# david-wb/tiny-diffusion

Measured on AMD Instinct MI355X. Metric: train images/s (q_sample+fwd+MSE+bwd+allreduce+Adam), MNIST 28x28 UNet fp32; 1000-step sample latency in `sample`, higher is better.
Workload: dtype f32; 1 GPU; diffusion.py unconditional MNIST 28x28 UNet, fp32, train step, batch 256/GPU (BASELINE.json configs[1]); global_batch=256, per_gpu_batch=256, parallelism=dp1

## Files before the change

### tiny_diffusion_amd/csrc/conv3x3_wino.hip

```cpp
#include "internal.h"
#include "conv_shared.h"


constexpr int WT = 64;
constexpr int WN = 64;
constexpr int WK = 8;
constexpr int A_ST = 16 * WT * WK;
constexpr int B_ST = 16 * WN * WK;
constexpr int STAGE = A_ST + B_ST;

struct WinoArgs {
  const float* in;
  const float* u;
  const float* bias;
  float* out;
  const float* out_scale;
  const float* out_shift;
  float* stats;
  int B, H, W, Cin, Cout, th, tw, NT, tilesN, M;
  float rcp_tpi, rcp_tw;
  int per;
  int compact;
  unsigned long long* stamps;
};

constexpr int OLD = 68;
constexpr int TAB_OFF = 2 * STAGE;
typedef unsigned u32x4 __attribute__((ext_vector_type(4)));

template <int EPI, int XH = -1>
__device__ __forceinline__ void wino_epilogue(const WinoArgs& a, float* out, const float* bias, f32x16 (&acc)[16], float* smem,
                                              int tblk, int n0, int wm, int wn, int l31, int half, int tid,
                                              const f32x4* xin = nullptr) {
#if defined(__HIP_DEVICE_COMPILE__)
  const unsigned* tab = reinterpret_cast<const unsigned*>(smem + TAB_OFF);
  const int cl = wn * 32 + l31, col = n0 + cl;
  const float bv = bias ? bias[col] : 0.f;
  float osc = 1.f, osh = 0.f;
  if (EPI == EPI_BNRELU) { osc = a.out_scale[col]; osh = a.out_shift[col]; }
  float csum = 0.f, cnt = 0.f;
  float* ot = smem;
  f32x4 pv[8];
#pragma unroll
  for (int r = 0; r < 16; ++r) {
    if (XH >= 0 && (r & 3) == 0) {
#pragma unroll
      for (int p = 0; p < 8; ++p) pv[p] = xin[(p * 4 + (r >> 2)) * 64];
    }
    auto M = [&](int p) { return XH >= 0 && (p >> 3) != XH ? pv[p & 7][r & 3] : acc[p][r]; };
    float s0[4], s1[4];
#pragma unroll
    for (int nu = 0; nu < 4; ++nu) {
      s0[nu] = M(0 + nu) + M(4 + nu) + M(8 + nu);
      s1[nu] = M(4 + nu) - M(8 + nu) - M(12 + nu);
    }
    float y[4] = {s0[0] + s0[1] + s0[2], s0[1] - s0[2] - s0[3], s1[0] + s1[1] + s1[2], s1[1] - s1[2] - s1[3]};
    const int tl = wm * 32 + (r & 3) + 8 * (r >> 2) + 4 * half;
    const unsigned m = tab[2 * tl + 1];
#pragma unroll
    for (int q = 0; q < 4; ++q) {
      float val = y[q] + bv;
      if (EPI == EPI_BNRELU) val = fmaxf(fmaf(val, osc, osh), 0.f);
      const bool ok = (m >> q) & 1u;
      if (XH < 0) ot[(tl * 4 + q) * OLD + cl] = val;
      csum += ok ? val : 0.f;
      cnt += ok ? 1.f : 0.f;
      y[q] = ok ? val : 0.f;
    }
    acc[0][r] = y[0]; acc[1][r] = y[1]; acc[4][r] = y[2]; acc[5][r] = y[3];
    acc[2][r] = (m & 1u) ? 1.f : 0.f;
    acc[3][r] = (m & 2u) ? 1.f : 0.f;
    acc[6][r] = (m & 4u) ? 1.f : 0.f;
    acc[7][r] = (m & 8u) ? 1.f : 0.f;
  }
  if (XH >= 0) {
    __syncthreads();
#pragma unroll
    for (int r = 0; r < 16; ++r) {
      const int tl = wm * 32 + (r & 3) + 8 * (r >> 2) + 4 * half;
      ot[(tl * 4 + 0) * OLD + cl] = acc[0][r]; ot[(tl * 4 + 1) * OLD + cl] = acc[1][r];
      ot[(tl * 4 + 2) * OLD + cl] = acc[4][r]; ot[(tl * 4 + 3) * OLD + cl] = acc[5][r];
    }
  }
  __syncthreads();
  {
    const auto rsrc_out = __builtin_amdgcn_make_buffer_rsrc(out, 0, (int)((int64_t)a.M * a.Cout * 4), 0x00020000);
    const int c4 = (tid & 15) * 4, q = (tid >> 4) & 3;
    const unsigned qoff = (unsigned)((((q >> 1) * a.W + (q & 1)) * a.Cout + n0 + c4) * 4);
    const uint2* tab2 = reinterpret_cast<const uint2*>(tab);
    const float* src = ot + (tid >> 4) * OLD + c4;
#pragma unroll
    for (int i = 0; i < 16; ++i) {
      const uint2 e = tab2[4 * i + (tid >> 6)];
      const unsigned off = ((e.y >> q) & 1u) ? e.x + qoff : 0x80000000u;
      const f32x4 v = *reinterpret_cast<const f32x4*>(src + i * 16 * OLD);
      __builtin_amdgcn_raw_buffer_store_b128(__builtin_bit_cast(u32x4, v), rsrc_out, off, 0, 0);
    }
  }
  if (EPI == EPI_STATS) {
    float* red = smem + 256 * OLD;
    const float s = csum + __shfl_xor(csum, 32, 64);
    const float n = cnt + __shfl_xor(cnt, 32, 64);
    if (half == 0) { red[wm * 64 + cl] = s; red[128 + wm * 64 + cl] = n; }
    __syncthreads();
    if (tid < 64) {
      const float ts = red[tid] + red[64 + tid];
      const float tn = red[128 + tid] + red[192 + tid];
      red[256 + tid] = tn > 0.f ? ts / tn : 0.f;
      a.stats[((size_t)tblk * 2 + 0) * a.Cout + n0 + tid] = ts;
    }
    __syncthreads();
    const float mean = red[256 + cl];
    float q = 0.f;
#pragma unroll
    for (int r = 0; r < 16; ++r) {
      const float d0 = acc[0][r] - mean, d1 = acc[1][r] - mean, d2 = acc[4][r] - mean, d3 = acc[5][r] - mean;
      q = fmaf(d0 * acc[2][r], d0, q); q = fmaf(d1 * acc[3][r], d1, q);
      q = fmaf(d2 * acc[6][r], d2, q); q = fmaf(d3 * acc[7][r], d3, q);
    }
    q += __shfl_xor(q, 32, 64);
    __syncthreads();
    if (half == 0) red[wm * 64 + cl] = q;
    __syncthreads();
    if (tid < 64) a.stats[((size_t)tblk * 2 + 1) * a.Cout + n0 + tid] = red[tid] + red[64 + tid];
  }
#endif
}

#if defined(__HIP_DEVICE_COMPILE__)
__device__ __forceinline__ float s_add(float x, float y) { float r; asm("v_add_f32 %0, %1, %2" : "=v"(r) : "v"(x), "v"(y)); return r; }
__device__ __forceinline__ float s_sub(float x, float y) { float r; asm("v_sub_f32 %0, %1, %2" : "=v"(r) : "v"(x), "v"(y)); return r; }
__device__ __forceinline__ f32x4 add4(f32x4 x, f32x4 y) { return f32x4{s_add(x[0], y[0]), s_add(x[1], y[1]), s_add(x[2], y[2]), s_add(x[3], y[3])}; }
__device__ __forceinline__ f32x4 sub4(f32x4 x, f32x4 y) { return f32x4{s_sub(x[0], y[0]), s_sub(x[1], y[1]), s_sub(x[2], y[2]), s_sub(x[3], y[3])}; }
#endif

__device__ __forceinline__ int div_rcp(int n, int d, float r, int* rem) {
  int q = (int)((float)n * r);
  int m = n - q * d;
  if (m < 0) { --q; m += d; }
  else if (m >= d) { ++q; m -= d; }
  *rem = m;
  return q;
}

template <int EPI, bool SPLITK, bool ROWS>
__global__ void __launch_bounds__(256)
conv3x3_wino_kernel(WinoArgs a) {
#if defined(__HIP_DEVICE_COMPILE__)
  static_assert(!ROWS || (!SPLITK && EPI != EPI_BNRELU), "the row split serves the training launches only");
  typedef __attribute__((address_space(3))) void* lds_ptr_t;
  extern __shared__ __attribute__((aligned(16))) float smem[];
  const unsigned long long t_entry = a.stamps ? __builtin_amdgcn_s_memrealtime() : 0ull;
  const int tid = threadIdx.x;
  const int lane = tid & 63;
  const int wave = __builtin_amdgcn_readfirstlane(tid >> 6);
  const int l31 = lane & 31, half = lane >> 5;
  const int wm = ROWS ? wave & 1 : wave >> 1, wn = ROWS ? wave >> 1 : wave & 1;
  const int xb = blockIdx.x / (8 * a.tilesN), xr = blockIdx.x % (8 * a.tilesN);
  const int tblk = a.compact ? (int)blockIdx.x / a.tilesN : xb * 8 + (xr & 7);
  const int nblk = a.compact ? (int)blockIdx.x - tblk * a.tilesN : xr >> 3;
  const int T0 = tblk * WT;
  if (T0 >= a.NT) return;
  const int n0 = nblk * WN;
  const int tpi = a.th * a.tw;

  if (tid < WT) {
    const int T = T0 + tid;
    const bool tv = T < a.NT;
    int rem, tx;
    const int b = div_rcp(T, tpi, a.rcp_tpi, &rem);
    const int ty = div_rcp(rem, a.tw, a.rcp_tw, &tx);
    const bool r1 = 2 * ty + 1 < a.H, c1 = 2 * tx + 1 < a.W;
    unsigned* tab = reinterpret_cast<unsigned*>(smem + TAB_OFF);
    tab[2 * tid] = tv ? (unsigned)(((b * a.H + 2 * ty) * a.W + 2 * tx) * a.Cout * 4) : 0u;
    tab[2 * tid + 1] = tv ? (1u | (c1 ? 2u : 0u) | (r1 ? 4u : 0u) | (r1 && c1 ? 8u : 0u)) : 0u;
  }

  const auto rsrc_in = __builtin_amdgcn_make_buffer_rsrc(const_cast<float*>(a.in), 0, (int)((int64_t)a.M * a.Cin * 4), 0x00020000);
  const auto rsrc_u = __builtin_amdgcn_make_buffer_rsrc(const_cast<float*>(a.u), 0, a.Cout * 16 * a.Cin * 4, 0x00020000);
  constexpr unsigned OOB = 0x80000000u;
  unsigned a_off[4][2];
#pragma unroll
  for (int g = 0; g < 2; ++g) {
    const int T = T0 + g * 32 + (lane >> 1);
    const bool tv = T < a.NT;
    int rem, tx;
    const int b = div_rcp(T, tpi, a.rcp_tpi, &rem);
    const int ty = div_rcp(rem, a.tw, a.rcp_tw, &tx);
#pragma unroll
    for (int j = 0; j < 4; ++j) {
      const int px = 4 * wave + j;
      const int ih = 2 * ty - 1 + (px >> 2), iw = 2 * tx - 1 + (px & 3);
      const bool ok = tv && (unsigned)ih < (unsigned)a.H && (unsigned)iw < (unsigned)a.W;
      a_off[j][g] = ok ? (unsigned)((((b * a.H + ih) * a.W + iw) * a.Cin + (lane & 1) * 4) * 4) : OOB;
    }
  }
  const unsigned u_base = (unsigned)(nblk * (a.Cin / WK)) * (unsigned)(B_ST * 4) + (unsigned)(wave * 8 * 1024 + lane * 16);

  const int s0 = SPLITK ? (int)blockIdx.y * a.per : 0;
  const int ns = SPLITK ? min(a.per, a.Cin / WK - s0) : a.Cin / WK;
  auto piece = [&](int i, int buf, int k) {
    const int sc = s0 + (k < ns ? k : ns - 1);
    float* Ab = smem + buf * STAGE;
    float* Bb = Ab + A_ST;
    if (i < 8)
      __builtin_amdgcn_raw_ptr_buffer_load_lds(rsrc_u, (lds_ptr_t)(Bb + (wave * 8 + i) * 256), 16, u_base + i * 1024,
                                               (unsigned)sc * (unsigned)(B_ST * 4), 0, 0);
    else
      __builtin_amdgcn_raw_ptr_buffer_load_lds(rsrc_in, (lds_ptr_t)(Ab + (4 * wave + ((i - 8) >> 1)) * 512 + ((i - 8) & 1) * 256), 16,
                                               a_off[(i - 8) >> 1][(i - 8) & 1], (unsigned)(sc * WK * 4), 0, 0);
  };

  constexpr bool PEEL = !SPLITK && EPI != EPI_BNRELU;
  f32x16 acc[16];
  const f32x16 zero16 = {0.f, 0.f, 0.f, 0.f, 0.f, 0.f, 0.f, 0.f, 0.f, 0.f, 0.f, 0.f, 0.f, 0.f, 0.f, 0.f};
  if (!PEEL) {
#pragma unroll
    for (int p = 0; p < 16; ++p)
#pragma unroll
      for (int r = 0; r < 16; ++r) acc[p][r] = 0.f;
  }

#pragma unroll
  for (int i = 0; i < 16; ++i) piece(i, 0, 0);
  unsigned long long t_issued = 0, t_landed = 0, t_loop = 0, c_loop = 0;
  if constexpr (ROWS) {
    static_assert(4 * 8 * 16 * 64 == 2 * STAGE, "the exchange fills the ring");
#pragma unroll
    for (int i = 0; i < 8; ++i) piece(i, 1, 1);
    if (a.stamps) t_issued = __builtin_amdgcn_s_memrealtime();
    asm volatile("s_waitcnt vmcnt(8) lgkmcnt(0)\n\ts_barrier" ::: "memory");
    if (a.stamps) { t_landed = __builtin_amdgcn_s_memrealtime(); c_loop = __builtin_amdgcn_s_memtime(); }
    auto body = [&](auto Hc) {
      constexpr int H = decltype(Hc)::value;
      f32x4 d[12], v[8], t[4], bq[5], nbq[2];
      const int lofs = wm * 256 + l31 * 8 + half * 4;
      auto trow = [&](int x, int c) {
        if (H == 0) t[c] = x == 0 ? sub4(d[c], d[8 + c]) : add4(d[4 + c], d[8 + c]);
        else t[c] = x == 0 ? sub4(d[4 + c], d[c]) : sub4(d[c], d[8 + c]);
      };
      auto vcol = [&](int x, int c) {
        f32x4& o = v[4 * x + c];
        if (c == 0) o = sub4(t[0], t[2]);
        else if (c == 1) o = add4(t[1], t[2]);
        else if (c == 2) o = sub4(t[2], t[1]);
        else o = sub4(t[1], t[3]);
      };
      constexpr int RA = 0, RB = H == 0 ? 2 : 1, RC = H == 0 ? 1 : 2;
      {
        const float* Ab = smem + 4 * H * 512 + lofs;
        const float* Bb = smem + A_ST + 8 * H * 512 + l31 * 8 + half * 4;
#pragma unroll
        for (int c = 0; c < 4; ++c) {
          d[4 * RA + c] = *reinterpret_cast<const f32x4*>(Ab + (4 * RA + c) * 512);
          d[4 * RB + c] = *reinterpret_cast<const f32x4*>(Ab + (4 * RB + c) * 512);
        }
        nbq[0] = *reinterpret_cast<const f32x4*>(Bb);
        nbq[1] = *reinterpret_cast<const f32x4*>(Bb + 256);
#pragma unroll
        for (int c = 0; c < 4; ++c) d[4 * RC + c] = *reinterpret_cast<const f32x4*>(Ab + (4 * RC + c) * 512);
#pragma unroll
        for (int c = 0; c < 4; ++c) trow(0, c);
#pragma unroll
        for (int c = 0; c < 4; ++c) vcol(0, c);
      }
      auto stage = [&](auto first_c, int s) {
        constexpr bool FIRST = decltype(first_c)::value;
        const int cb = s & 1;
        const float* Bb = smem + cb * STAGE + A_ST + 8 * H * 512 + l31 * 8 + half * 4;
        const float* An = smem + (cb ^ 1) * STAGE + 4 * H * 512 + lofs;
        const float* Bn = smem + (cb ^ 1) * STAGE + A_ST + 8 * H * 512 + l31 * 8 + half * 4;
        bq[0] = nbq[0]; bq[1] = nbq[1];
        __builtin_amdgcn_sched_barrier(0);
#pragma unroll
        for (int g = 0; g < 16; ++g) {
          const int cur = g % 5, pp = g >> 1, ai = 8 * (g & 1) + pp;
          if (FIRST) acc[ai] = __builtin_amdgcn_mfma_f32_32x32x2f32(v[pp][0], bq[cur][0], zero16, 0, 0, 0);
          else acc[ai] = __builtin_amdgcn_mfma_f32_32x32x2f32(v[pp][0], bq[cur][0], acc[ai], 0, 0, 0);
          if (g < 8) piece(8 + g, cb ^ 1, s + 1);
          if (g == 10) bq[4] = *reinterpret_cast<const f32x4*>(Bb + 14 * 256);
          if (g == 11) bq[0] = *reinterpret_cast<const f32x4*>(Bb + 15 * 256);
          if (g == 12) {
            asm volatile("s_waitcnt vmcnt(0) lgkmcnt(0)\n\ts_barrier" ::: "memory");
#pragma unroll
            for (int c = 0; c < 4; ++c) {
              d[4 * RA + c] = *reinterpret_cast<const f32x4*>(An + (4 * RA + c) * 512);
              d[4 * RB + c] = *reinterpret_cast<const f32x4*>(An + (4 * RB + c) * 512);
            }
          }
          if (g == 13) {
#pragma unroll
            for (int c = 0; c < 4; ++c) d[4 * RC + c] = *reinterpret_cast<const f32x4*>(An + (4 * RC + c) * 512);
          }
          if (g == 14) {
#pragma unroll
            for (int c = 0; c < 4; ++c) trow(0, c);
          }
          if (g == 15) { vcol(0, 2); vcol(0, 3); }
          __builtin_amdgcn_sched_barrier(0);
          acc[ai] = __builtin_amdgcn_mfma_f32_32x32x2f32(v[pp][1], bq[cur][1], acc[ai], 0, 0, 0);
          if (g < 2) { trow(1, 2 * g); trow(1, 2 * g + 1); }
          else if (g < 4) { vcol(1, 2 * g - 4); vcol(1, 2 * g - 3); }
          else if (g >= 12) piece(2 * (g - 12), cb, s + 2);
          __builtin_amdgcn_sched_barrier(0);
          acc[ai] = __builtin_amdgcn_mfma_f32_32x32x2f32(v[pp][2], bq[cur][2], acc[ai], 0, 0, 0);
          if (g < 12) bq[(g + 2) % 5] = *reinterpret_cast<const f32x4*>(Bb + (g + 2) * 256);
          if (g == 12) { nbq[0] = *reinterpret_cast<const f32x4*>(Bn); nbq[1] = *reinterpret_cast<const f32x4*>(Bn + 256); }
          if (g == 14) { vcol(0, 0); vcol(0, 1); }
          if (g == 15) piece(7, cb, s + 2);
          __builtin_amdgcn_sched_barrier(0);
          acc[ai] = __builtin_amdgcn_mfma_f32_32x32x2f32(v[pp][3], bq[cur][3], acc[ai], 0, 0, 0);
          if (g >= 12 && g < 15) piece(2 * (g - 12) + 1, cb, s + 2);
          __builtin_amdgcn_sched_barrier(0);
        }
      };
      stage(std::true_type{}, 0);
      for (int s = 1; s < ns; ++s) stage(std::false_type{}, s);
      asm volatile("s_waitcnt vmcnt(0) lgkmcnt(0)\n\ts_barrier" ::: "memory");
      if (a.stamps) { t_loop = __builtin_amdgcn_s_memrealtime(); c_loop = __builtin_amdgcn_s_memtime() - c_loop; }
      {
        f32x4* xo = reinterpret_cast<f32x4*>(smem) + (2 * (1 - H) + wm) * 2048 + lane;
#pragma unroll
        for (int pp = 0; pp < 8; ++pp)
#pragma unroll
          for (int r4 = 0; r4 < 4; ++r4) {
            const f32x16& x = acc[8 * (1 - H) + pp];
            xo[(pp * 4 + r4) * 64] = f32x4{x[4 * r4], x[4 * r4 + 1], x[4 * r4 + 2], x[4 * r4 + 3]};
          }
      }
      __syncthreads();
      wino_epilogue<EPI, H>(a, a.out, a.bias, acc, smem, tblk, n0, wm, H, l31, half, tid,
                            reinterpret_cast<const f32x4*>(smem) + wave * 2048 + lane);
    };
    if (wn) body(std::integral_constant<int, 1>{});
    else body(std::integral_constant<int, 0>{});
  } else {
    f32x4 d[16], v[16], t1[4], t2[4], t3[4];
    auto xop = [&](int q) {
      const int r = q >> 3, k = q & 7, c = k & 3;
      if (k < 4) {
        if (r == 0) t1[c] = add4(d[4 + c], d[8 + c]);
        else if (r == 1) t2[c] = sub4(d[8 + c], d[4 + c]);
        else t3[c] = sub4(d[4 + c], d[12 + c]);
      } else {
        f32x4(&t)[4] = r == 0 ? t1 : r == 1 ? t2 : t3;
        f32x4& o = v[4 * (r + 1) + c];
        if (c == 0) o = sub4(t[0], t[2]);
        else if (c == 1) o = add4(t[1], t[2]);
        else if (c == 2) o = sub4(t[2], t[1]);
        else o = sub4(t[1], t[3]);
      }
    };
    {
#pragma unroll
      for (int i = 0; i < 8; ++i) piece(i, 1, 1);
      if (a.stamps) t_issued = __builtin_amdgcn_s_memrealtime();
      asm volatile("s_waitcnt vmcnt(8) lgkmcnt(0)\n\ts_barrier" ::: "memory");
      if (a.stamps) { t_landed = __builtin_amdgcn_s_memrealtime(); c_loop = __builtin_amdgcn_s_memtime(); }
      f32x4 bq[5], nbq[2];
      {
        const float* Ab = smem + wm * 256 + l31 * 8 + half * 4;
        const float* Bb = smem + A_ST + wn * 256 + l31 * 8 + half * 4;
#pragma unroll
        for (int c = 0; c < 4; ++c) { d[c] = *reinterpret_cast<const f32x4*>(Ab + c * 512); d[8 + c] = *reinterpret_cast<const f32x4*>(Ab + (8 + c) * 512); }
        nbq[0] = *reinterpret_cast<const f32x4*>(Bb);
        nbq[1] = *reinterpret_cast<const f32x4*>(Bb + 512);
#pragma unroll
        for (int c = 0; c < 4; ++c) { d[4 + c] = *reinterpret_cast<const f32x4*>(Ab + (4 + c) * 512); d[12 + c] = *reinterpret_cast<const f32x4*>(Ab + (12 + c) * 512); }
        f32x4 t0[4];
#pragma unroll
        for (int c = 0; c < 4; ++c) t0[c] = sub4(d[c], d[8 + c]);
        v[0] = sub4(t0[0], t0[2]); v[1] = add4(t0[1], t0[2]); v[2] = sub4(t0[2], t0[1]); v[3] = sub4(t0[1], t0[3]);
      }
      auto stage = [&](auto first_c, int s) {
        constexpr bool FIRST = decltype(first_c)::value;
        const int cb = s & 1;
        const float* Bb = smem + cb * STAGE + A_ST + wn * 256 + l31 * 8 + half * 4;
        const float* An = smem + (cb ^ 1) * STAGE + wm * 256 + l31 * 8 + half * 4;
        const float* Bn = smem + (cb ^ 1) * STAGE + A_ST + wn * 256 + l31 * 8 + half * 4;
        bq[0] = nbq[0]; bq[1] = nbq[1];
        __builtin_amdgcn_sched_barrier(0);
#pragma unroll
        for (int p = 0; p < 16; ++p) {
          const int cur = p % 5;
          if (FIRST) acc[p] = __builtin_amdgcn_mfma_f32_32x32x2f32(v[p][0], bq[cur][0], zero16, 0, 0, 0);
          else acc[p] = __builtin_amdgcn_mfma_f32_32x32x2f32(v[p][0], bq[cur][0], acc[p], 0, 0, 0);
          if (p < 8) piece(8 + p, cb ^ 1, s + 1);
          if (p == 10) bq[4] = *reinterpret_cast<const f32x4*>(Bb + 14 * 512);
          if (p == 11) bq[0] = *reinterpret_cast<const f32x4*>(Bb + 15 * 512);
          if (p == 12) {
            asm volatile("s_waitcnt vmcnt(0) lgkmcnt(0)\n\ts_barrier" ::: "memory");
#pragma unroll
            for (int c = 0; c < 4; ++c) { d[c] = *reinterpret_cast<const f32x4*>(An + c * 512); d[8 + c] = *reinterpret_cast<const f32x4*>(An + (8 + c) * 512); }
          }
          if (p == 13) {
#pragma unroll
            for (int c = 0; c < 4; ++c) d[4 + c] = *reinterpret_cast<const f32x4*>(An + (4 + c) * 512);
          }
          if (p == 14) {
#pragma unroll
            for (int c = 0; c < 4; ++c) t1[c] = sub4(d[c], d[8 + c]);
          }
          if (p == 15) { v[2] = sub4(t1[2], t1[1]); v[3] = sub4(t1[1], t1[3]); }
          __builtin_amdgcn_sched_barrier(0);
          acc[p] = __builtin_amdgcn_mfma_f32_32x32x2f32(v[p][1], bq[cur][1], acc[p], 0, 0, 0);
          if (p < 12) { xop(2 * p); xop(2 * p + 1); }
          else piece(2 * (p - 12), cb, s + 2);
          __builtin_amdgcn_sched_barrier(0);
          acc[p] = __builtin_amdgcn_mfma_f32_32x32x2f32(v[p][2], bq[cur][2], acc[p], 0, 0, 0);
          if (p < 12) bq[(p + 2) % 5] = *reinterpret_cast<const f32x4*>(Bb + (p + 2) * 512);
          if (p == 12) { nbq[0] = *reinterpret_cast<const f32x4*>(Bn); nbq[1] = *reinterpret_cast<const f32x4*>(Bn + 512); }
          if (p == 13) {
#pragma unroll
            for (int c = 0; c < 4; ++c) d[12 + c] = *reinterpret_cast<const f32x4*>(An + (12 + c) * 512);
          }
          if (p == 14) { v[0] = sub4(t1[0], t1[2]); v[1] = add4(t1[1], t1[2]); }
          if (p == 15) piece(7, cb, s + 2);
          __builtin_amdgcn_sched_barrier(0);
          acc[p] = __builtin_amdgcn_mfma_f32_32x32x2f32(v[p][3], bq[cur][3], acc[p], 0, 0, 0);
          if (p >= 12 && p < 15) piece(2 * (p - 12) + 1, cb, s + 2);
          __builtin_amdgcn_sched_barrier(0);
        }
      };
      if (PEEL) stage(std::true_type{}, 0);
      for (int s = PEEL ? 1 : 0; s < ns; ++s) stage(std::false_type{}, s);
      asm volatile("s_waitcnt vmcnt(0) lgkmcnt(0)\n\ts_barrier" ::: "memory");
    }
    if (a.stamps) { t_loop = __builtin_amdgcn_s_memrealtime(); c_loop = __builtin_amdgcn_s_memtime() - c_loop; }
    if (SPLITK)
      wino_epilogue<EPI_PLAIN>(a, a.out + (size_t)blockIdx.y * (size_t)a.M * a.Cout, nullptr, acc, smem, tblk, n0, wm, wn, l31, half, tid);
    else
      wino_epilogue<EPI>(a, a.out, a.bias, acc, smem, tblk, n0, wm, wn, l31, half, tid);
  }
  if (a.stamps && tid == 0) {
    asm volatile("s_waitcnt vmcnt(0)" ::: "memory");
    unsigned long long* o = a.stamps + 8 * ((size_t)blockIdx.y * gridDim.x + blockIdx.x);
    o[0] = t_entry; o[1] = t_issued; o[2] = t_landed; o[3] = t_loop; o[4] = __builtin_amdgcn_s_memrealtime();
    o[5] = c_loop;
    o[6] = __builtin_amdgcn_s_getreg(4 | (0 << 6) | (31 << 11));
    o[7] = __builtin_amdgcn_s_getreg(20 | (0 << 6) | (3 << 11)) & 0xf;
  }
#endif
}

__global__ void __launch_bounds__(512) pack_wino_batch_kernel(TdxWinoPackBatch b) {
  int u = 0;
  while (u + 1 < b.count && (int)blockIdx.x >= b.start[u + 1]) ++u;
  const int cin = b.cin[u], cout = b.cout[u], cin_real = b.cin_real[u];
  const int blk = blockIdx.x - b.start[u];
  const int nkb = cin / 8;
  const int cb = blk / nkb, kb = blk - cb * nkb;
  const int cl = threadIdx.x >> 3, k8 = threadIdx.x & 7;
  const int co = cb * 64 + cl, ci = kb * 8 + k8;
  float g[9];
#pragma unroll
  for (int tap = 0; tap < 9; ++tap) g[tap] = ci < cin_real ? b.w[u][((size_t)co * cin_real + ci) * 9 + tap] : 0.f;
  float gg[4][3], U[16];
#pragma unroll
  for (int c = 0; c < 3; ++c) {
    gg[0][c] = g[c];
    gg[1][c] = 0.5f * (g[c] + g[3 + c] + g[6 + c]);
    gg[2][c] = 0.5f * (g[c] - g[3 + c] + g[6 + c]);
    gg[3][c] = g[6 + c];
  }
#pragma unroll
  for (int r = 0; r < 4; ++r) {
    U[r * 4 + 0] = gg[r][0];
    U[r * 4 + 1] = 0.5f * (gg[r][0] + gg[r][1] + gg[r][2]);
    U[r * 4 + 2] = 0.5f * (gg[r][0] - gg[r][1] + gg[r][2]);
    U[r * 4 + 3] = gg[r][2];
  }
  if (b.uf[u]) {
    float* dst = b.uf[u] + (((size_t)cb * nkb + kb) * 16) * 512 + cl * 8 + k8;
#pragma unroll
    for (int p = 0; p < 16; ++p) dst[p * 512] = U[p];
  }
  if (b.ud[u]) {
    float* dst = b.ud[u] + (((size_t)(ci >> 6) * (cout / 8) + (co >> 3)) * 16) * 512 + (ci & 63) * 8 + (co & 7);
    constexpr int ps = 512;
#pragma unroll
    for (int p = 0; p < 16; ++p) {
      const int xi = p >> 2, nu = p & 3;
      const int sx = xi == 0 ? 3 : xi == 3 ? 0 : xi, sn = nu == 0 ? 3 : nu == 3 ? 0 : nu;
      dst[p * ps] = U[sx * 4 + sn];
    }
  }
}

static int wino_tile_rows(int H, int W) {
  const int th = (H + 1) / 2, tw = (W + 1) / 2;
  if (!(H & 1) && !(W & 1)) return 4 * WT;
  if (WT % (th * tw) == 0) return (WT / (th * tw)) * H * W;
  return 0;
}

extern "C" int tdx_conv3x3_wino_ok(int B, int H, int W, int cin, int cout) {
  if (B <= 0 || H <= 0 || W <= 0 || cin <= 0 || cout <= 0 || cin % WK || cout % WN) return 0;
  if (!wino_tile_rows(H, W)) return 0;
  const int64_t M = (int64_t)B * H * W;
  return M * cin * 4 < (1ll << 31) && M * cout * 4 < (1ll << 31) && (int64_t)cout * 16 * cin * 4 < (1ll << 31) &&
         (int64_t)B * ((H + 1) / 2) * ((W + 1) / 2) + 64 < (1ll << 24);
}

extern "C" int tdx_conv3x3_wino_stat_tile_rows(int B, int H, int W) { (void)B; return wino_tile_rows(H, W); }
extern "C" int tdx_conv3x3_wino_stat_tiles(int B, int H, int W) {
  const int th = (H + 1) / 2, tw = (W + 1) / 2;
  return cdiv((int64_t)B * th * tw, WT);
}

int tdx_pack_conv3x3_wino_pad(const float* w_oihw, float* u_fwd, float* u_dgrad, int cout, int cin_real, int cin,
                              tdx_stream_t stream);

int tdx_pack_conv3x3_wino_batch(TdxWinoPackBatch* b, tdx_stream_t stream) {
  if (!b || b->count <= 0 || b->count > TDX_PACK_MAX) return TDX_E_BADARG;
  int blocks = 0;
  for (int u = 0; u < b->count; ++u) {
    if (!b->w[u] || b->cin_real[u] <= 0 || b->cin_real[u] > b->cin[u] || b->cin[u] % 64 || b->cout[u] % 64) return TDX_E_BADARG;
    b->start[u] = blocks;
    blocks += (b->cin[u] / 8) * (b->cout[u] / 64);
  }
  pack_wino_batch_kernel<<<blocks, 512, 0, to_stream(stream)>>>(*b);
  TDX_CHECK_LAUNCH();
  return 0;
}

int tdx_pack_conv3x3_wino_pad(const float* w_oihw, float* u_fwd, float* u_dgrad, int cout, int cin_real, int cin,
                              tdx_stream_t stream) {
  if (!w_oihw || cout <= 0 || cin <= 0 || cin_real <= 0 || cin_real > cin) return TDX_E_BADARG;
  if (cin % 64 || cout % 64) return TDX_E_SHAPE;
  if (!u_fwd && !u_dgrad) return 0;
  TdxWinoPackBatch b{};
  b.count = 1;
  b.w[0] = w_oihw; b.uf[0] = u_fwd; b.ud[0] = u_dgrad; b.cout[0] = cout; b.cin[0] = cin; b.cin_real[0] = cin_real;
  return tdx_pack_conv3x3_wino_batch(&b, stream);
}

extern "C" int tdx_pack_conv3x3_wino(const float* w_oihw, float* u_fwd, float* u_dgrad, int cout, int cin,
                                     tdx_stream_t stream) {
  return tdx_pack_conv3x3_wino_pad(w_oihw, u_fwd, u_dgrad, cout, cin, cin, stream);
}

int tdx_conv3x3_wino_launch(const float* in, const float* u, const float* bias, float* out, int B, int H, int W,
                            int cin, int cout, int flags, const float* out_scale, const float* out_shift,
                            float* stats_partial, int splits, int per, tdx_stream_t stream) {
  if (!in || !u || !out) return TDX_E_BADARG;
  if (!tdx_conv3x3_wino_ok(B, H, W, cin, cout)) return TDX_E_SHAPE;
  if (flags & ~(TDX_CONV_OUT_BNRELU | TDX_CONV_OUT_STATS)) return TDX_E_BADARG;
  if ((flags & TDX_CONV_OUT_BNRELU) && (!out_scale || !out_shift)) return TDX_E_BADARG;
  if ((flags & TDX_CONV_OUT_STATS) && (!stats_partial || (flags & TDX_CONV_OUT_BNRELU))) return TDX_E_BADARG;
  if (splits < 1 || (splits > 1 && (per < 1 || (int64_t)per * (splits - 1) >= cin / WK))) return TDX_E_BADARG;
  WinoArgs a{};
  a.in = in; a.u = u; a.bias = bias; a.out = out; a.out_scale = out_scale; a.out_shift = out_shift;
  a.stats = stats_partial;
  a.B = B; a.H = H; a.W = W; a.Cin = cin; a.Cout = cout;
  a.th = (H + 1) / 2; a.tw = (W + 1) / 2;
  a.NT = B * a.th * a.tw;
  a.rcp_tpi = 1.0f / (float)(a.th * a.tw); a.rcp_tw = 1.0f / (float)a.tw;
  a.tilesN = cout / WN;
  a.M = B * H * W;
  a.per = per;
  a.compact = cdiv(a.NT, WT) < 64;
  const dim3 grid(a.compact ? cdiv(a.NT, WT) * a.tilesN : (cdiv(a.NT, WT) + 7) / 8 * 8 * a.tilesN, splits);
  a.stamps = g_knobs.conv_stamp == 3 && g_tdx_diag_buffer && (size_t)grid.x * grid.y * 64 <= g_tdx_diag_bytes
                 ? reinterpret_cast<unsigned long long*>(g_tdx_diag_buffer) : nullptr;
  const size_t lds = (size_t)2 * STAGE * sizeof(float) + WT * 2 * sizeof(unsigned);
  hipStream_t st = to_stream(stream);
#define TDX_WINO_LAUNCH(EPI_, SPL_, ROWS_)                                                                       \
  do {                                                                                                           \
    auto kern = conv3x3_wino_kernel<EPI_, SPL_, ROWS_>;                                                          \
    static bool attr_set = false;                                                                                \
    if (!attr_set) {                                                                                             \
      hipError_t e = hipFuncSetAttribute(reinterpret_cast<const void*>(kern),                                    \
                                         hipFuncAttributeMaxDynamicSharedMemorySize, (int)lds);                  \
      if (e != hipSuccess) return (int)e;                                                                        \
      attr_set = true;                                                                                           \
    }                                                                                                            \
    kern<<<grid, 256, lds, st>>>(a);                                                                             \
  } while (0)
  const bool rows = g_knobs.wino_rows && cin / WK >= g_knobs.wino_rows_min_stages;
  if (splits > 1) TDX_WINO_LAUNCH(EPI_PLAIN, true, false);
  else if (flags & TDX_CONV_OUT_BNRELU) TDX_WINO_LAUNCH(EPI_BNRELU, false, false);
  else if (flags & TDX_CONV_OUT_STATS) {
    if (rows) TDX_WINO_LAUNCH(EPI_STATS, false, true);
    else TDX_WINO_LAUNCH(EPI_STATS, false, false);
  } else if (rows) TDX_WINO_LAUNCH(EPI_PLAIN, false, true);
  else TDX_WINO_LAUNCH(EPI_PLAIN, false, false);
#undef TDX_WINO_LAUNCH
  TDX_CHECK_LAUNCH();
  return 0;
}

extern "C" int tdx_conv3x3_fwd_wino(const float* in, const float* u, const float* bias, float* out, int B, int H, int W,
                                    int cin, int cout, int flags, const float* out_scale, const float* out_shift,
                                    float* stats_partial, tdx_stream_t stream) {
  return tdx_conv3x3_wino_launch(in, u, bias, out, B, H, W, cin, cout, flags, out_scale, out_shift, stats_partial, 1, 0,
                                 stream);
}

constexpr int GT8 = 8;
constexpr int XS_F = GT8 * 16 * 64;
constexpr int ES_F = GT8 * 4 * 64;
constexpr int WST_F = XS_F + ES_F;
constexpr int WNST = 3;
constexpr int WG_MAX_CHUNK = 1024;
constexpr int WG_XCH_F = 4 * 8 * 16 * 64;
constexpr size_t WG_LDS = 131072;
static_assert((size_t)WNST * WST_F * 4 + (size_t)WG_MAX_CHUNK * 4 <= WG_LDS && (size_t)WG_XCH_F * 4 <= WG_LDS, "LDS");

struct WinoWgArgs {
  const float* in;
  const float* dy;
  float* slabs;
  int B, H, W, Cin, Cout, th, tw, NT, M;
  int tilesCo, tilesCi, chunk;
  unsigned long long* stamps;
};

#if defined(__HIP_DEVICE_COMPILE__)
__device__ __forceinline__ unsigned long long wg_lanes16(unsigned m) {
  unsigned long long r;
  asm("s_bitreplicate_b64_b32 %0, %1" : "=s"(r) : "s"(m));
  asm("s_bitreplicate_b64_b32 %0, %1" : "=s"(r) : "s"((unsigned)r));
  asm("s_bitreplicate_b64_b32 %0, %1" : "=s"(r) : "s"((unsigned)r));
  asm("s_bitreplicate_b64_b32 %0, %1" : "=s"(r) : "s"((unsigned)r));
  return r;
}
__device__ __forceinline__ unsigned wg_sel(unsigned long long mask, unsigned x, unsigned y) {
  unsigned r;
  asm("v_cndmask_b32_e64 %0, %1, %2, %3" : "=v"(r) : "v"(y), "v"(x), "s"(mask));
  return r;
}
#endif

__global__ void __launch_bounds__(256)
conv3x3_wgrad_wino_kernel(WinoWgArgs a) {
// ... 318 lines not shown
```

Measured before the change: 27840 images/s.

## Restructure Winograd epilogue exchange and issue first loads before index setup

The Winograd conv epilogue in the row-split path gets a new LDS layout. Each wave writes its own output tile region instead of using a second barrier-separated pass, and partial-sum prefetch is double-buffered. Row pairs are processed as 2-wide vectors, and a FULL specialization drops mask handling when tiles are fully interior and H and W are even. The kernel prologue now issues the first 8 async loads before building the tile table and address offsets, so address arithmetic overlaps memory latency, and the a_off computation is simplified per wave row. This adds template variants, which may increase code size and register pressure.

```diff
diff --git a/tiny_diffusion_amd/csrc/conv3x3_wino.hip b/tiny_diffusion_amd/csrc/conv3x3_wino.hip
--- a/tiny_diffusion_amd/csrc/conv3x3_wino.hip
+++ b/tiny_diffusion_amd/csrc/conv3x3_wino.hip
@@ -26,9 +26,11 @@
 
 constexpr int OLD = 68;
 constexpr int TAB_OFF = 2 * STAGE;
+constexpr int XREG = 2 * STAGE / 4;
+constexpr int XQ = XREG / 4;
 typedef unsigned u32x4 __attribute__((ext_vector_type(4)));
 
-template <int EPI, int XH = -1>
+template <int EPI, int XH = -1, bool FULL = false>
 __device__ __forceinline__ void wino_epilogue(const WinoArgs& a, float* out, const float* bias, f32x16 (&acc)[16], float* smem,
                                               int tblk, int n0, int wm, int wn, int l31, int half, int tid,
                                               const f32x4* xin = nullptr) {
@@ -39,48 +41,72 @@
   float osc = 1.f, osh = 0.f;
   if (EPI == EPI_BNRELU) { osc = a.out_scale[col]; osh = a.out_shift[col]; }
   float csum = 0.f, cnt = 0.f;
+  constexpr bool RX = XH >= 0;
   float* ot = smem;
-  f32x4 pv[8];
-#pragma unroll
-  for (int r = 0; r < 16; ++r) {
-    if (XH >= 0 && (r & 3) == 0) {
-#pragma unroll
-      for (int p = 0; p < 8; ++p) pv[p] = xin[(p * 4 + (r >> 2)) * 64];
-    }
-    auto M = [&](int p) { return XH >= 0 && (p >> 3) != XH ? pv[p & 7][r & 3] : acc[p][r]; };
-    float s0[4], s1[4];
+  float* own = smem + (RX ? (2 * XH + wm) * XREG : 0);
+  auto red = [&](int slot, int g, int c) -> float* {
+    return RX ? smem + (2 * (c >> 5) + g) * XREG + XQ / 2 + slot * 32 + (c & 31) : smem + 256 * OLD + (2 * slot + g) * 64 + c;
+  };
+  float* means = RX ? smem + XQ / 2 + 128 : smem + 256 * OLD + 384;
+  f32x4 pv[2][8];
+  if (RX) {
+#pragma unroll
+    for (int p = 0; p < 8; ++p) pv[0][p] = xin[p * 64];
+  }
+  constexpr int RW = EPI == EPI_BNRELU ? 1 : 2;
+  typedef float rowv __attribute__((ext_vector_type(RW)));
+#pragma unroll
+  for (int r = 0; r < 16; r += RW) {
+    if (RX && (r & 3) == 0 && r < 12) {
+#pragma unroll
+      for (int p = 0; p < 8; ++p) pv[((r >> 2) + 1) & 1][p] = xin[(((r >> 2) + 1) * 8 + p) * 64];
+    }
+    auto M = [&](int p) {
+      rowv v;
+#pragma unroll
+      for (int e = 0; e < RW; ++e) v[e] = RX && (p >> 3) != XH ? pv[(r >> 2) & 1][p & 7][(r & 3) + e] : acc[p][r + e];
+      return v;
+    };
+    rowv s0[4], s1[4], bv2;
+#pragma unroll
+    for (int e = 0; e < RW; ++e) bv2[e] = bv;
 #pragma unroll
     for (int nu = 0; nu < 4; ++nu) {
       s0[nu] = M(0 + nu) + M(4 + nu) + M(8 + nu);
       s1[nu] = M(4 + nu) - M(8 + nu) - M(12 + nu);
     }
-    float y[4] = {s0[0] + s0[1] + s0[2], s0[1] - s0[2] - s0[3], s1[0] + s1[1] + s1[2], s1[1] - s1[2] - s1[3]};
-    const int tl = wm * 32 + (r & 3) + 8 * (r >> 2) + 4 * half;
-    const unsigned m = tab[2 * tl + 1];
-#pragma unroll
-    for (int q = 0; q < 4; ++q) {
-      float val = y[q] + bv;
-      if (EPI == EPI_BNRELU) val = fmaxf(fmaf(val, osc, osh), 0.f);
-      const bool ok = (m >> q) & 1u;
-      if (XH < 0) ot[(tl * 4 + q) * OLD + cl] = val;
-      csum += ok ? val : 0.f;
-      cnt += ok ? 1.f : 0.f;
-      y[q] = ok ? val : 0.f;
-    }
-    acc[0][r] = y[0]; acc[1][r] = y[1]; acc[4][r] = y[2]; acc[5][r] = y[3];
-    acc[2][r] = (m & 1u) ? 1.f : 0.f;
-    acc[3][r] = (m & 2u) ? 1.f : 0.f;
-    acc[6][r] = (m & 4u) ? 1.f : 0.f;
-    acc[7][r] = (m & 8u) ? 1.f : 0.f;
-  }
-  if (XH >= 0) {
-    __syncthreads();
-#pragma unroll
-    for (int r = 0; r < 16; ++r) {
-      const int tl = wm * 32 + (r & 3) + 8 * (r >> 2) + 4 * half;
-      ot[(tl * 4 + 0) * OLD + cl] = acc[0][r]; ot[(tl * 4 + 1) * OLD + cl] = acc[1][r];
-      ot[(tl * 4 + 2) * OLD + cl] = acc[4][r]; ot[(tl * 4 + 3) * OLD + cl] = acc[5][r];
-    }
+    const rowv y2[4] = {s0[0] + s0[1] + s0[2] + bv2, s0[1] - s0[2] - s0[3] + bv2, s1[0] + s1[1] + s1[2] + bv2,
+                         s1[1] - s1[2] - s1[3] + bv2};
+#pragma unroll
+    for (int e = 0; e < RW; ++e) {
+      const int re = r + e;
+      const int tl = wm * 32 + (re & 3) + 8 * (re >> 2) + 4 * half;
+      const unsigned m = FULL ? 15u : tab[2 * tl + 1];
+      float y[4];
+#pragma unroll
+      for (int q = 0; q < 4; ++q) {
+        float val = y2[q][e];
+        if (EPI == EPI_BNRELU) val = fmaxf(fmaf(val, osc, osh), 0.f);
+        const bool ok = (m >> q) & 1u;
+        if (RX) own[(re >> 2) * XQ + (((re & 3) + 4 * half) * 4 + q) * 32 + l31] = val;
+        else ot[(tl * 4 + q) * OLD + cl] = val;
+        csum += ok ? val : 0.f;
+        cnt += ok ? 1.f : 0.f;
+        y[q] = ok ? val : 0.f;
+      }
+      acc[0][re] = y[0]; acc[1][re] = y[1]; acc[4][re] = y[2]; acc[5][re] = y[3];
+      if (!FULL) {
+        acc[2][re] = (m & 1u) ? 1.f : 0.f;
+        acc[3][re] = (m & 2u) ? 1.f : 0.f;
+        acc[6][re] = (m & 4u) ? 1.f : 0.f;
+        acc[7][re] = (m & 8u) ? 1.f : 0.f;
+      }
+    }
+  }
+  if (EPI == EPI_STATS) {
+    const float s = csum + __shfl_xor(csum, 32, 64);
+    const float n = cnt + __shfl_xor(cnt, 32, 64);
+    if (half == 0) { *red(0, wm, cl) = s; *red(1, wm, cl) = n; }
   }
   __syncthreads();
   {
@@ -88,41 +114,39 @@
     const int c4 = (tid & 15) * 4, q = (tid >> 4) & 3;
     const unsigned qoff = (unsigned)((((q >> 1) * a.W + (q & 1)) * a.Cout + n0 + c4) * 4);
     const uint2* tab2 = reinterpret_cast<const uint2*>(tab);
-    const float* src = ot + (tid >> 4) * OLD + c4;
+    const float* src = RX ? smem + 2 * (c4 >> 5) * XREG + (tid >> 4) * 32 + (c4 & 31) : ot + (tid >> 4) * OLD + c4;
 #pragma unroll
     for (int i = 0; i < 16; ++i) {
       const uint2 e = tab2[4 * i + (tid >> 6)];
       const unsigned off = ((e.y >> q) & 1u) ? e.x + qoff : 0x80000000u;
-      const f32x4 v = *reinterpret_cast<const f32x4*>(src + i * 16 * OLD);
+      const f32x4 v = *reinterpret_cast<const f32x4*>(src + (RX ? (i >> 3) * XREG + ((i & 7) >> 1) * XQ + (i & 1) * 512 : i * 16 * OLD));
       __builtin_amdgcn_raw_buffer_store_b128(__builtin_bit_cast(u32x4, v), rsrc_out, off, 0, 0);
     }
   }
   if (EPI == EPI_STATS) {
-    float* red = smem + 256 * OLD;
-    const float s = csum + __shfl_xor(csum, 32, 64);
-    const float n = cnt + __shfl_xor(cnt, 32, 64);
-    if (half == 0) { red[wm * 64 + cl] = s; red[128 + wm * 64 + cl] = n; }
+    if (tid < 64) {
+      const float ts = *red(0, 0, tid) + *red(0, 1, tid);
+      const float tn = *red(1, 0, tid) + *red(1, 1, tid);
+      means[tid] = tn > 0.f ? ts / tn : 0.f;
+      a.stats[((size_t)tblk * 2 + 0) * a.Cout + n0 + tid] = ts;
+    }
     __syncthreads();
-    if (tid < 64) {
-      const float ts = red[tid] + red[64 + tid];
-      const float tn = red[128 + tid] + red[192 + tid];
-      red[256 + tid] = tn > 0.f ? ts / tn : 0.f;
-      a.stats[((size_t)tblk * 2 + 0) * a.Cout + n0 + tid] = ts;
-    }
-    __syncthreads();
-    const float mean = red[256 + cl];
+    const float mean = means[cl];
     float q = 0.f;
 #pragma unroll
     for (int r = 0; r < 16; ++r) {
       const float d0 = acc[0][r] - mean, d1 = acc[1][r] - mean, d2 = acc[4][r] - mean, d3 = acc[5][r] - mean;
-      q = fmaf(d0 * acc[2][r], d0, q); q = fmaf(d1 * acc[3][r], d1, q);
-      q = fmaf(d2 * acc[6][r], d2, q); q = fmaf(d3 * acc[7][r], d3, q);
+      if (FULL) {
+        q = fmaf(d0, d0, q); q = fmaf(d1, d1, q); q = fmaf(d2, d2, q); q = fmaf(d3, d3, q);
+      } else {
+        q = fmaf(d0 * acc[2][r], d0, q); q = fmaf(d1 * acc[3][r], d1, q);
+        q = fmaf(d2 * acc[6][r], d2, q); q = fmaf(d3 * acc[7][r], d3, q);
+      }
     }
     q += __shfl_xor(q, 32, 64);
+    if (half == 0) *red(2, wm, cl) = q;
     __syncthreads();
-    if (half == 0) red[wm * 64 + cl] = q;
-    __syncthreads();
-    if (tid < 64) a.stats[((size_t)tblk * 2 + 1) * a.Cout + n0 + tid] = red[tid] + red[64 + tid];
+    if (tid < 64) a.stats[((size_t)tblk * 2 + 1) * a.Cout + n0 + tid] = *red(2, 0, tid) + *red(2, 1, tid);
   }
 #endif
 }
@@ -164,38 +188,11 @@
   const int n0 = nblk * WN;
   const int tpi = a.th * a.tw;
 
-  if (tid < WT) {
-    const int T = T0 + tid;
-    const bool tv = T < a.NT;
-    int rem, tx;
-    const int b = div_rcp(T, tpi, a.rcp_tpi, &rem);
-    const int ty = div_rcp(rem, a.tw, a.rcp_tw, &tx);
-    const bool r1 = 2 * ty + 1 < a.H, c1 = 2 * tx + 1 < a.W;
-    unsigned* tab = reinterpret_cast<unsigned*>(smem + TAB_OFF);
-    tab[2 * tid] = tv ? (unsigned)(((b * a.H + 2 * ty) * a.W + 2 * tx) * a.Cout * 4) : 0u;
-    tab[2 * tid + 1] = tv ? (1u | (c1 ? 2u : 0u) | (r1 ? 4u : 0u) | (r1 && c1 ? 8u : 0u)) : 0u;
-  }
-
   const auto rsrc_in = __builtin_amdgcn_make_buffer_rsrc(const_cast<float*>(a.in), 0, (int)((int64_t)a.M * a.Cin * 4), 0x00020000);
   const auto rsrc_u = __builtin_amdgcn_make_buffer_rsrc(const_cast<float*>(a.u), 0, a.Cout * 16 * a.Cin * 4, 0x00020000);
   constexpr unsigned OOB = 0x80000000u;
+  const unsigned u_base = (unsigned)(nblk * (a.Cin / WK)) * (unsigned)(B_ST * 4) + (unsigned)(wave * 8 * 1024 + lane * 16);
   unsigned a_off[4][2];
-#pragma unroll
-  for (int g = 0; g < 2; ++g) {
-    const int T = T0 + g * 32 + (lane >> 1);
-    const bool tv = T < a.NT;
-    int rem, tx;
-    const int b = div_rcp(T, tpi, a.rcp_tpi, &rem);
-    const int ty = div_rcp(rem, a.tw, a.rcp_tw, &tx);
-#pragma unroll
-    for (int j = 0; j < 4; ++j) {
-      const int px = 4 * wave + j;
-      const int ih = 2 * ty - 1 + (px >> 2), iw = 2 * tx - 1 + (px & 3);
-      const bool ok = tv && (unsigned)ih < (unsigned)a.H && (unsigned)iw < (unsigned)a.W;
-      a_off[j][g] = ok ? (unsigned)((((b * a.H + ih) * a.W + iw) * a.Cin + (lane & 1) * 4) * 4) : OOB;
-    }
-  }
-  const unsigned u_base = (unsigned)(nblk * (a.Cin / WK)) * (unsigned)(B_ST * 4) + (unsigned)(wave * 8 * 1024 + lane * 16);
 
   const int s0 = SPLITK ? (int)blockIdx.y * a.per : 0;
   const int ns = SPLITK ? min(a.per, a.Cin / WK - s0) : a.Cin / WK;
@@ -210,8 +207,43 @@
       __builtin_amdgcn_raw_ptr_buffer_load_lds(rsrc_in, (lds_ptr_t)(Ab + (4 * wave + ((i - 8) >> 1)) * 512 + ((i - 8) & 1) * 256), 16,
                                                a_off[(i - 8) >> 1][(i - 8) & 1], (unsigned)(sc * WK * 4), 0, 0);
   };
-
   constexpr bool PEEL = !SPLITK && EPI != EPI_BNRELU;
+  if (PEEL) {
+#pragma unroll
+    for (int i = 0; i < 8; ++i) piece(i, 0, 0);
+    __builtin_amdgcn_sched_barrier(0);
+  }
+
+  if (tid < WT) {
+    const int T = T0 + tid;
+    const bool tv = T < a.NT;
+    int rem, tx;
+    const int b = div_rcp(T, tpi, a.rcp_tpi, &rem);
+    const int ty = div_rcp(rem, a.tw, a.rcp_tw, &tx);
+    const bool r1 = 2 * ty + 1 < a.H, c1 = 2 * tx + 1 < a.W;
+    unsigned* tab = reinterpret_cast<unsigned*>(smem + TAB_OFF);
+    tab[2 * tid] = tv ? (unsigned)(((b * a.H + 2 * ty) * a.W + 2 * tx) * a.Cout * 4) : 0u;
+    tab[2 * tid + 1] = tv ? (1u | (c1 ? 2u : 0u) | (r1 ? 4u : 0u) | (r1 && c1 ? 8u : 0u)) : 0u;
+  }
+
+#pragma unroll
+  for (int g = 0; g < 2; ++g) {
+    const int T = T0 + g * 32 + (lane >> 1);
+    const bool tv = T < a.NT;
+    int rem, tx;
+    const int b = div_rcp(T, tpi, a.rcp_tpi, &rem);
+    const int ty = div_rcp(rem, a.tw, a.rcp_tw, &tx);
+    const int ih = 2 * ty - 1 + wave;
+    const bool rok = tv && (unsigned)ih < (unsigned)a.H;
+    const int rowpx = (b * a.H + ih) * a.W;
+#pragma unroll
+    for (int j = 0; j < 4; ++j) {
+      const int iw = 2 * tx - 1 + j;
+      const bool ok = rok && (unsigned)iw < (unsigned)a.W;
+      a_off[j][g] = ok ? (unsigned)(((rowpx + iw) * a.Cin + (lane & 1) * 4) * 4) : OOB;
+    }
+  }
+
   f32x16 acc[16];
   const f32x16 zero16 = {0.f, 0.f, 0.f, 0.f, 0.f, 0.f, 0.f, 0.f, 0.f, 0.f, 0.f, 0.f, 0.f, 0.f, 0.f, 0.f};
   if (!PEEL) {
@@ -222,7 +254,7 @@
   }
 
 #pragma unroll
-  for (int i = 0; i < 16; ++i) piece(i, 0, 0);
+  for (int i = PEEL ? 8 : 0; i < 16; ++i) piece(i, 0, 0);
   unsigned long long t_issued = 0, t_landed = 0, t_loop = 0, c_loop = 0;
   if constexpr (ROWS) {
     static_assert(4 * 8 * 16 * 64 == 2 * STAGE, "the exchange fills the ring");
@@ -319,18 +351,22 @@
       asm volatile("s_waitcnt vmcnt(0) lgkmcnt(0)\n\ts_barrier" ::: "memory");
       if (a.stamps) { t_loop = __builtin_amdgcn_s_memrealtime(); c_loop = __builtin_amdgcn_s_memtime() - c_loop; }
       {
-        f32x4* xo = reinterpret_cast<f32x4*>(smem) + (2 * (1 - H) + wm) * 2048 + lane;
+        f32x4* xo = reinterpret_cast<f32x4*>(smem + (2 * (1 - H) + wm) * XREG) + lane;
 #pragma unroll
         for (int pp = 0; pp < 8; ++pp)
 #pragma unroll
           for (int r4 = 0; r4 < 4; ++r4) {
             const f32x16& x = acc[8 * (1 - H) + pp];
-            xo[(pp * 4 + r4) * 64] = f32x4{x[4 * r4], x[4 * r4 + 1], x[4 * r4 + 2], x[4 * r4 + 3]};
+            xo[(r4 * 8 + pp) * 64] = f32x4{x[4 * r4], x[4 * r4 + 1], x[4 * r4 + 2], x[4 * r4 + 3]};
           }
       }
       __syncthreads();
-      wino_epilogue<EPI, H>(a, a.out, a.bias, acc, smem, tblk, n0, wm, H, l31, half, tid,
-                            reinterpret_cast<const f32x4*>(smem) + wave * 2048 + lane);
+      if (EPI == EPI_STATS && !((a.H | a.W) & 1) && T0 + WT <= a.NT)
+        wino_epilogue<EPI, H, true>(a, a.out, a.bias, acc, smem, tblk, n0, wm, H, l31, half, tid,
+                                    reinterpret_cast<const f32x4*>(smem + wave * XREG) + lane);
+      else
+        wino_epilogue<EPI, H>(a, a.out, a.bias, acc, smem, tblk, n0, wm, H, l31, half, tid,
+                              reinterpret_cast<const f32x4*>(smem + wave * XREG) + lane);
     };
     if (wn) body(std::integral_constant<int, 1>{});
     else body(std::integral_constant<int, 0>{});
```

Measured after the change: 28140 images/s, median of 6. 1.1% higher.
